# hydradarpa/kalman-hydra

Measured on AMD Instinct MI355X. Metric: frames/sec (Brox flow + EKF update) at 1024^2, higher is better.
Workload: dtype f32 (flow, renders) / f64 (EKF sums and state)

## Files before the change

include/hydra_mi.h:

```cpp
#ifndef HYDRA_MI_H
#define HYDRA_MI_H

#include <stdint.h>

#ifdef __cplusplus
extern "C" {
#endif

#define HM_OK 0
#define HM_ERR_ARG (-1)
#define HM_ERR_HIP (-2)
#define HM_ERR_STATE (-3)
#define HM_ERR_NUMERIC (-4)

const char *hm_last_error(void);
const char *hm_version(void);
int hm_device_count(void);

int hm_dev_alloc(int device, uint64_t bytes, void **out);
int hm_dev_free(int device, void *ptr);
int hm_dev_upload(int device, void *dst, const void *src, uint64_t bytes);
int hm_dev_download(int device, void *dst, const void *src, uint64_t bytes);
int hm_copy_stream_create(int device, void **stream_out);
int hm_copy_stream_destroy(int device, void *stream);
// ... 88 lines not shown
int hm_ms_newton_finish(void *worker, double *X, int *newton_iterations);
int hm_ms_worker_attach(void *worker, hm_ctx_t ctx);
int hm_newton_dev_start(hm_ctx_t h, int N, int n_bars, const int32_t *bars, const double *l0, double kappa, double M,
                        double dt, int maxiter, double tol, const double *X);
int hm_newton_dev_finish(hm_ctx_t h, double *X, int *newton_iterations);
int hm_update_arm_newton(hm_ctx_t h, void *worker, int n_bars, const int32_t *bars, const double *l0, double kappa,
                         double M, double dt, int maxiter, double tol);
int hm_update_arm_cov(hm_ctx_t h, double eps_F);
int hm_predict_take(hm_ctx_t h, const double *X, int n_bars, const int32_t *bars, const double *l0, double kappa,
                    double a, double s, double eps_F);
int hm_cov_predict(hm_ctx_t h, const double *W_in, int n_bars, const int32_t *bars, const double *blocks,
                   double a, double s, double eps_F, double *W_out);
int hm_ms_predict(hm_ctx_t h, int n_bars, const int32_t *bars, const double *l0, double kappa, double M, double dt,
                  int maxiter, double tol, double eps_F, double *X, int *newton_iterations, int prefactor);
int hm_update_last_error(hm_ctx_t h, const double *X, double err[4]);
int hm_chain_project(hm_ctx_t h);
int hm_prepare_mask(hm_ctx_t h, const uint8_t *d_y_m);
int hm_update_arm_mask(hm_ctx_t h, const uint8_t *d_y_m);
int hm_update_tail(hm_ctx_t h, double *Hzc, double *gains);
int hm_chain_states(hm_ctx_t h, double *predicted, double *projected, int *newton_iterations, int *moved);
int hm_ctx_tune(hm_ctx_t h, const char *key, int value);
int hm_ctx_tune64(hm_ctx_t h, const char *key, int64_t value);
int hm_ctx_sync(hm_ctx_t h);
void *hm_ctx_stream(hm_ctx_t h);

typedef struct hm_smooth *hm_smooth_t;
int hm_smooth_create(hm_ctx_t ctx, int capacity, int n_bars, const int32_t *bars, const double *l0, double kappa,
                     double a, double s, double eps_F, hm_smooth_t *out);
int hm_smooth_destroy(hm_smooth_t sm);
int hm_smooth_record(hm_smooth_t sm, const double *X);
// ... 142 lines not shown
```

kalman-hydra_amd/_lib.py:

```python
import ctypes
import os

import numpy as np

_HERE = os.path.dirname(os.path.abspath(__file__))
SO_PATH = os.environ.get("HYDRA_MI_SO") or os.path.join(_HERE, "libhydra_mi.so")

c_f32p = ctypes.POINTER(ctypes.c_float)
c_f64p = ctypes.POINTER(ctypes.c_double)
c_u8p = ctypes.POINTER(ctypes.c_uint8)
c_i32p = ctypes.POINTER(ctypes.c_int32)
c_vp = ctypes.c_void_p

SIGNATURES = {
    "hm_last_error": (ctypes.c_char_p, []),
    "hm_version": (ctypes.c_char_p, []),
    "hm_device_count": (ctypes.c_int, []),
    "hm_dev_alloc": (ctypes.c_int, [ctypes.c_int, ctypes.c_uint64, ctypes.POINTER(c_vp)]),
    "hm_dev_free": (ctypes.c_int, [ctypes.c_int, c_vp]),
    "hm_dev_upload": (ctypes.c_int, [ctypes.c_int, c_vp, c_vp, ctypes.c_uint64]),
    "hm_dev_download": (ctypes.c_int, [ctypes.c_int, c_vp, c_vp, ctypes.c_uint64]),
    "hm_copy_stream_create": (ctypes.c_int, [ctypes.c_int, ctypes.POINTER(c_vp)]),
    "hm_copy_stream_destroy": (ctypes.c_int, [ctypes.c_int, c_vp]),
    "hm_copy_stream_sync": (ctypes.c_int, [ctypes.c_int, c_vp]),
# ... 39 lines not shown
    "hm_render": (ctypes.c_int, [c_vp, c_vp, c_vp, c_vp, c_vp, c_vp]),
    "hm_initjacobian": (ctypes.c_int, [c_vp, c_vp, ctypes.c_int]),
    "hm_jz": (ctypes.c_int, [c_vp, c_vp, ctypes.c_int, c_f64p, c_f64p]),
    "hm_j": (ctypes.c_int, [c_vp, c_vp, ctypes.c_double, ctypes.c_int, ctypes.c_int, c_f64p]),
    "hm_jz_multi": (ctypes.c_int, [c_vp, c_vp, ctypes.c_int, c_vp, ctypes.c_int, c_vp, c_vp]),
    "hm_j_multi": (ctypes.c_int, [c_vp, c_vp, ctypes.c_double, ctypes.c_int, c_vp, c_vp, ctypes.c_int, c_vp, c_vp, c_vp]),
    "hm_error": (ctypes.c_int, [c_vp, c_vp, ctypes.c_int, c_f64p, c_vp, c_vp]),
    "hm_measure": (ctypes.c_int, [c_vp, c_vp, ctypes.c_double, ctypes.c_int, c_vp, c_vp, c_vp]),
    "hm_update_begin": (ctypes.c_int, [c_vp, c_vp, c_vp]),
    "hm_update_step": (ctypes.c_int, [c_vp, c_vp, ctypes.c_double, ctypes.c_int, c_vp, c_vp, c_f64p]),
    "hm_update_cov": (ctypes.c_int, [c_vp, ctypes.c_int, c_vp]),
    "hm_update_prefactor": (ctypes.c_int, [c_vp]),
    "hm_update_run": (ctypes.c_int, [c_vp, c_vp, c_vp, ctypes.c_double, ctypes.c_int, ctypes.c_int, ctypes.c_double,
                                     ctypes.POINTER(ctypes.c_int), c_vp, c_vp, c_vp, c_vp]),
    "hm_update_last_error": (ctypes.c_int, [c_vp, c_vp, c_f64p]),
    "hm_cov_fetch": (ctypes.c_int, [c_vp, c_vp]),
    "hm_project_mask": (ctypes.c_int, [c_vp, c_vp, c_vp, c_vp]),
    "hm_cov_predict": (ctypes.c_int, [c_vp, c_vp, ctypes.c_int, c_vp, c_vp, ctypes.c_double, ctypes.c_double,
                                      ctypes.c_double, c_vp]),
    "hm_ms_newton": (ctypes.c_int, [ctypes.c_int, ctypes.c_int, c_vp, c_vp, ctypes.c_double, ctypes.c_double,
                                    ctypes.c_double, ctypes.c_int, ctypes.c_double, c_vp, ctypes.POINTER(ctypes.c_int)]),
    "hm_ms_worker_create": (ctypes.c_int, [ctypes.POINTER(c_vp)]),
    "hm_ms_worker_destroy": (ctypes.c_int, [c_vp]),
    "hm_ms_newton_start": (ctypes.c_int, [c_vp, ctypes.c_int, ctypes.c_int, c_vp, c_vp, ctypes.c_double, ctypes.c_double,
                                          ctypes.c_double, ctypes.c_int, ctypes.c_double, c_vp]),
    "hm_ms_newton_finish": (ctypes.c_int, [c_vp, c_vp, ctypes.POINTER(ctypes.c_int)]),
    "hm_ms_worker_attach": (ctypes.c_int, [c_vp, c_vp]),
    "hm_newton_dev_start": (ctypes.c_int, [c_vp, ctypes.c_int, ctypes.c_int, c_vp, c_vp, ctypes.c_double, ctypes.c_double,
                                           ctypes.c_double, ctypes.c_int, ctypes.c_double, c_vp]),
    "hm_newton_dev_finish": (ctypes.c_int, [c_vp, c_vp, ctypes.POINTER(ctypes.c_int)]),
# ... 223 lines not shown
```

kalman-hydra_amd/csrc/ctx.h:

```cpp
#pragma once
#include "hm_common.h"
#include "hm_types.h"
#include "host_block.h"
#include <chrono>
#include <cmath>
#include <condition_variable>
#include <functional>
#include <mutex>
#include <thread>
#include <vector>

struct Helper {
    std::thread th;
    std::mutex m;
    std::condition_variable cv;
    std::function<int()> job;
    bool posted = false, busy = false, quit = false;
    int rc = HM_OK;
    char err[512] = "";
    void run()
    {
        std::unique_lock<std::mutex> lk(m);
        for (;;) {
            cv.wait(lk, [&] { return quit || posted; });
// ... 273 lines not shown
    Armed armed;
    hipEvent_t ev_m0 = nullptr;
    bool upd_open = false;
    bool prefactored = false;
    bool last_err_valid = false;
    double last_err[4] = {0, 0, 0, 0};
    std::vector<double> last_err_X;
    long long run_ticket = 0;
    std::thread worker;
    bool worker_active = false;
    int worker_rc = HM_OK;
    char worker_err[512] = "";
    int chol_flow = 1, flow_wgs = 192;
    int flow_stall = 0;
    int speculate = 1;
    double *d_flowP = nullptr;
    unsigned *d_flowctl = nullptr;
    MaskState mask;
    Newton4State newton4;
    NewtonState newton;
    ChainState chain;
    SpringState sp;
    ArmedPrediction pn;
    QueuedPrediction pq;
    TailState tail;
    MultiState multi;
    ViewState view;
    BodyState body;
    StrainState strain;
    RecState rec;
// ... 134 lines not shown
        const int a = bars[2 * i], b = bars[2 * i + 1];
        const double dx = X[2 * a] - X[2 * b], dy = X[2 * a + 1] - X[2 * b + 1];
        const double l = std::sqrt(dx * dx + dy * dy);
        const double k = kappa * (1.0 - l0[i] / l), c = kappa * l0[i] / (l * l * l);
        blk[3 * i] = k + c * dx * dx; blk[3 * i + 1] = c * dx * dy; blk[3 * i + 2] = k + c * dy * dy;
    }
}

__attribute__((visibility("hidden"))) void ekf_queue_setup_all(hipStream_t st, const Mesh &m, const double *d_X, TriSetup *d_setup);
__attribute__((visibility("hidden"))) void ekf_queue_render(hipStream_t st, const Mesh &m, const double *d_X, const TriSetup *d_setup,
                                                            const Targets &out, const int *d_labels, int *d_ids);
__attribute__((visibility("hidden"))) int render_iter(hm_ctx *h, const double *dX, Targets t, bool with_err, int masked, bool regions, double deltaX);
__attribute__((visibility("hidden"))) int render_strips(const hm_ctx *h);
__attribute__((visibility("hidden"))) int render_error_sums(hm_ctx *h, const char *who, double err[4]);
__attribute__((visibility("hidden"))) int measure_dev(hm_ctx *h, const double *dX, bool ref_ready, double deltaX, int masked,
                                                      bool regions_ready = false, bool scatter = true);
__attribute__((visibility("hidden"))) int measure_on_device(hm_ctx *h, const double *X, double deltaX, int masked, bool scatter = true);
__attribute__((visibility("hidden"))) int queue_star_regions(hm_ctx *h, const double *dX, double deltaX, int masked);
__attribute__((visibility("hidden"))) int pool_grow(hm_ctx *h, const char *who);
__attribute__((visibility("hidden"))) int prior_inverse(hm_ctx *h, const double *W_prior, hipStream_t st = nullptr);
#ifdef HM_STAMP
__attribute__((visibility("hidden"))) int update_debug_stamps(long long *dev_ptr);
#endif
__attribute__((visibility("hidden"))) int ensure_stream2(hm_ctx *h);
__attribute__((visibility("hidden"))) int queue_outline(hm_ctx *h, const uint8_t *mask);
__attribute__((visibility("hidden"))) int prepare_mask(hm_ctx *h, const uint8_t *d_y_m);
__attribute__((visibility("hidden"))) int queue_predict_ahead(hm_ctx *h, const double *X, int n_bars, const int32_t *bars, const double *l0,
                                                              double kappa, double M, double dt, double eps_F, hipStream_t st);

static inline int pool_flag_queue(hm_ctx *h)
{
// ... 24 lines not shown
```

kalman-hydra_amd/csrc/dense_kernels.h:

```cpp
#pragma once
#include <hip/hip_runtime.h>
#include "hm_types.h"
#include "host_block.h"

#define TTT_PF 3

__device__ __forceinline__ double d_rsqrt(double d)
{
    const double r = __builtin_amdgcn_rsq(d);
    const double e = fma(-(d * r), r, 1.0);
#ifdef HM_RSQRT_ORDER2
    return fma(r * 0.5, e, r);
#else
    return fma(r, fma(e, 0.375, 0.5) * e, r);
#endif
}

__device__ __forceinline__ double d_readlane(double v, int lane)
{
    const int lo = __builtin_amdgcn_readlane(__double2loint(v), lane);
    const int hi = __builtin_amdgcn_readlane(__double2hiint(v), lane);
    return __hiloint2double(hi, lo);
}

// ... 449 lines not shown
            for (int j = threadIdx.x; j < n; j += 256) A[(size_t)row * n + j] = 0.0;
        return;
    }
    double acc = 0.0;
    for (int j = threadIdx.x; j < n; j += 256) {
        const double h = H[(size_t)row * n + j];
        A[(size_t)row * n + j] = invW0[(size_t)row * n + j] + h;
        acc += h * (X0[j] + -1.0 * X[j]);
    }
    for (int o = 32; o > 0; o >>= 1) acc += __shfl_down(acc, o, 64);
    if ((threadIdx.x & 63) == 0) s[threadIdx.x >> 6] = acc;
    __syncthreads();
    if (threadIdx.x == 0) A[(size_t)rhs_row * n + row] = Hz[row] - (((s[0] + s[1]) + s[2]) + s[3]);
}


__global__ __launch_bounds__(256) void k_iter_result(const double *__restrict__ step, int n, const double *__restrict__ partial,
                                                     int ntiles, const int *__restrict__ overflow,
                                                     const unsigned *__restrict__ flow_ctl, double *__restrict__ res, double ticket,
                                                     int delay_us)
{
    __shared__ double sp[RI_GROUPS * RI_NV];
    __shared__ double sums[RI_NV];
    const int t = threadIdx.x;
    const unsigned long long stamp = hb_stamp((long long)ticket);
    d_tile_partial_sums(partial, ntiles, sp, sums);
    __syncthreads();
    double v = 0.0;
    int slot = -1;
    if (t < 4) { slot = t; v = sums[t]; }
    else if (t == 4) { slot = 4; v = (double)*overflow; }
    else if (t == 5) { slot = 5; v = ticket; }
    else if (t == 6) { slot = 6; v = 0.0; }
    else if (t == 7) { slot = 7; v = (double)flow_ctl[1]; }
    else if (t == 8) { slot = 8; v = sums[4]; }
    else if (t == 9) { slot = 9; v = sums[5]; }
    if (delay_us > 0) {
        if (t == 9) { hb_put(res, n + 9, v, stamp); hb_flush(); }
        hb_delay(delay_us);
    }
    for (int i = t; i < n; i += 256) hb_put(res, i, step[i], stamp);
    if (slot >= 0) hb_put(res, n + slot, v, stamp);
    hb_flush();
}

__global__ __launch_bounds__(256) void k_gains(const double *__restrict__ W, const double *__restrict__ Hzc, int n,
                                               double *__restrict__ out)
{
    __shared__ double sm[3][4];
    const int row = blockIdx.x;
    double a0 = 0.0, a1 = 0.0, a2 = 0.0;
    for (int j = threadIdx.x; j < n; j += 256) {
        const double w = W[(size_t)row * n + j];
        const double *c = Hzc + (size_t)4 * j;
        a0 += w * c[0];
        a1 += w * (c[1] + c[2]);
// ... 81 lines not shown
```

kalman-hydra_amd/csrc/ekf.hip:

```cpp
#include "ctx.h"
#include "ekf_kernels.h"
#include <algorithm>
#include <cmath>
#include <cstring>
#include <set>
#include <utility>
#include <vector>

static hipError_t pool_alloc(hm_ctx *h, long long cap)
{
    const size_t pc = (size_t)cap;
    h->pool.cap = 0;
    hipError_t e = h->own.grow(&h->pool.live, (pc / 64 + 1) * sizeof(int));
    for (short2 **q : {&h->pool.xi, &h->pool.yi})
        if (e == hipSuccess) e = h->own.grow(q, pc * sizeof(short2));
    for (float **q : {&h->pool.xfx, &h->pool.xfy, &h->pool.yfx, &h->pool.yfy, &h->pool.vxfx, &h->pool.vyfy})
        if (e == hipSuccess) e = h->own.grow(q, pc * sizeof(float));
    if (e == hipSuccess) h->pool.cap = cap;
    return e;
}
int pool_grow(hm_ctx *h, const char *who)
{
    std::vector<int> area(h->N);
    HM_HIP(hipMemcpyAsync(area.data(), h->d_area, (size_t)h->N * sizeof(int), hipMemcpyDeviceToHost, h->stream));
// ... 144 lines not shown
        dev(&h->d_Wprior, nn);
        dev(&h->d_gain, n4 * 3 * sizeof(double));
        h->pin_n = 2 * (n4 + RES_HEAD + n4 * 4 + n4 * 3) + 2;
        if (e == hipSuccess) e = h->own.host_alloc(&h->pin, h->pin_n * sizeof(double), hipHostMallocCoherent);
        if (e == hipSuccess) memset(h->pin, 0, h->pin_n * sizeof(double));
        h->pin_scratch = (int *)(h->pin + h->pin_n - 2);
        h->resv.assign(n4 + RES_HEAD, 0.0);
        h->tail.v.assign(n4 * 7, 0.0);
        dev(&h->d_X0, n4 * sizeof(double));
        dev(&h->pool.hdr, (size_t)4 * N * sizeof(int));
        dev(&h->pool.overflow, sizeof(int));
        dev(&h->d_area, (size_t)N * sizeof(int));
        h->pool.area = h->d_area;
        if (e == hipSuccess) e = pool_alloc(h, (long long)8 * W * H);
        dev(&h->d_Xn, n4 * sizeof(double));
        for (Targets *t : {&h->ref, &h->P, &h->Q})
            if (e == hipSuccess) e = alloc_targets(h->own, *t, n);
    }
    if (e != hipSuccess) {
        hm_set_error("hm_ctx_create: device allocation failed: %s", hipGetErrorString(e));
        step(HM_ERR_HIP);
    }
    if (rc != HM_OK) {
        ctx_free(h);
        return rc;
    }
    h->h_partial.resize((size_t)h->red_blocks * 4);
    h->h_tpart.resize((size_t)h->ntiles * RI_NV);
    *out = h;
    return HM_OK;
// ... 29 lines not shown
    int step;
    void (*set)(hm_ctx *, long long);
    const char *must;
} tune_keys[] = {
    {"measure_split", 1, MEAS_VSPLIT_MAX, 1, TUNE_SET(vsplit), nullptr},
    {"edge_split", 1, MEAS_VSPLIT_MAX, 1, TUNE_SET(esplit), nullptr},
    {"chol_flow", 0, 1, 1, TUNE_SET(chol_flow), "must be 0 (one launch per block step) or 1 (one persistent launch)"},
    {"chol_flow_wgs", 2, 2048, 1, TUNE_SET(flow_wgs), "must be in 2..2048 (the chain workgroup and at least one task workgroup)"},
    {"render_rows", 8, 16, 8, TUNE_SET(render_rows), "must be 8 or 16"},
    {"chol_flow_stall", 0, 100000, 1, TUNE_SET(flow_stall), nullptr},
    {"result_delay", 0, 5000, 1, TUNE_SET(result_delay), "must be in 0..5000 (microseconds)"},
    {"tail_async", 0, 1, 1, TUNE_SET(tail.async), "must be 0 or 1"},
    {"tail_split", 0, 1, 1, TUNE_SET(tail.split), "must be 0 or 1"},
    {"newton_fail", 0, 1, 1, TUNE_SET(newton4.fail), "must be 0 or 1"},
    {"speculate", 0, 1, 1, TUNE_SET(speculate), "must be 0 or 1"},
    {"body_stats_cap", 1, BODY_STATS_CAP, 1, TUNE_SET(body.stats_cap), nullptr},
    {"deep_col_entries", DEEP_COL_ENTRIES_MIN, DEEP_COL_ENTRIES_MAX, 1, TUNE_SET(body.deep_col_entries), nullptr},
    {"body_rec_chunk", 0, INT32_MAX, 1, TUNE_SET(rec.chunk), "must be >= 0 (0: the default size)"},
    {"rec_tp_frames", 1, REC_TP_MAX, 1, TUNE_SET(rec.tp_frames), nullptr},
    {"rec_bl_frames", 1, REC_BL_MAX, 1, TUNE_SET(rec.bl_frames), nullptr},
    {"rec_res_frames", 1, REC_RES_MAX, 1, TUNE_SET(rec.res_frames), nullptr},
    {"rec_map_frames", 1, REC_MAP_MAX, 1, TUNE_SET(rec.map_frames), nullptr},
    {"rec_null_frames", 1, REC_NULL_MAX, 1, TUNE_SET(rec.null_frames), nullptr},
    {"rec_tm_frames", 1, REC_TM_MAX, 1, TUNE_SET(rec.tm_frames), nullptr},
    {"rec_gram_bytes", 64, REC_GRAM_BYTES_MAX, 64, TUNE_SET(rec.gram_bytes), "must be a multiple of 64 in 64..131008"},
    {"rec_scratch_bytes", 1, 1 << 30, 1, TUNE_SET(rec.scr_bytes), nullptr},
    {"rec_ev_bytes", 1, 1ll << 34, 1, TUNE_SET(rec.ev_bytes), nullptr},
};
#undef TUNE_SET
static const TuneKey *tune_find(const char *key)
// ... 122 lines not shown
    a.ref = h->ref;
    a.obs = obs_of(h, masked);
    a.X = dX;
    a.delta = deltaX;
    a.out = h->d_out;
    a.pool = h->pool;
    a.vsplit = h->vsplit;
    a.esplit = h->esplit;
    a.iZ = 1.0 / h->eps_Z; a.iJ = 1.0 / h->eps_J; a.iM = 1.0 / h->eps_M;
    a.cfgs = h->d_cfgs;
    a.ubox = h->d_ubox;
    a.tmask = h->d_tmask;
    a.tlist = h->d_tlist;
    a.tcount = h->d_tcount;
    a.tmask_stride = TMASK_STRIDE;
}

static int state_upload(hm_ctx *h, const double *X)
{
    HM_HIP(hipMemcpyAsync(h->d_X, X, (size_t)4 * h->N * sizeof(double), hipMemcpyHostToDevice, h->stream));
    return HM_OK;
}

static int render_dev(hm_ctx *h, const double *dX, Targets t)
{
    const Mesh m = mesh_of(h);
    hipLaunchKernelGGL(k_setup_all, dim3(hm_cdiv(h->T, 64)), dim3(64), 0, h->stream, m, dX, h->d_setup);
    hipLaunchKernelGGL((k_render<0>), dim3(hm_cdiv(h->W, EKF_TILE), hm_cdiv(h->H, EKF_TILE)), dim3(EKF_TILE, EKF_TILE), 0,
                       h->stream, m, dX, h->d_setup, t, (const int *)nullptr, (int *)nullptr);
    HM_HIP(hipGetLastError());
// ... 275 lines not shown
    const int n = h->W * h->H;
    if (fx) HM_HIP(hipMemcpyAsync(fx, h->P.fx, (size_t)n * sizeof(float), hipMemcpyDeviceToHost, h->stream));
    if (fy) HM_HIP(hipMemcpyAsync(fy, h->P.fy, (size_t)n * sizeof(float), hipMemcpyDeviceToHost, h->stream));
    return render_error_sums(h, "hm_error", err);
}

int queue_star_regions(hm_ctx *h, const double *dX, double deltaX, int masked)
{
    MeasureArgs a;
    measure_args(h, dX, deltaX, masked, a);
    hipLaunchKernelGGL(k_star_regions, dim3(h->N), dim3(REGION_NT), 0, h->stream, a, h->d_area);
    HM_HIP(hipGetLastError());
    return HM_OK;
}

int measure_dev(hm_ctx *h, const double *dX, bool ref_ready, double deltaX, int masked, bool regions_ready, bool scatter)
{
    if (!ref_ready) {
        HM_TRY(render_iter(h, dX, h->ref, false, masked, !regions_ready, deltaX));
        regions_ready = true;
    }
    MeasureArgs a;
    measure_args(h, dX, deltaX, masked, a);
    if (!regions_ready) hipLaunchKernelGGL(k_star_regions, dim3(h->N), dim3(REGION_NT), 0, h->stream, a, h->d_area);
    hipLaunchKernelGGL(k_measure_vertex, dim3(h->N, h->vsplit), dim3(MEAS_NT), 0, h->stream, a,
                       (const TriSetup *)h->d_cfgs, (const int4 *)h->d_ubox, (const unsigned *)h->d_tmask);
    if (h->E > 0) hipLaunchKernelGGL(k_measure_edge, dim3(h->E, h->esplit), dim3(MEAS_NT), 0, h->stream, a);
    if (scatter) {
        ScatterArgs s = {h->d_out, h->d_edges, h->N, h->E, h->vsplit, h->esplit, h->eps_Z, h->eps_J, h->eps_M, deltaX, h->d_HTH, h->d_Hz, h->d_Hzc};
        hipLaunchKernelGGL(k_hth_scatter, dim3(hm_cdiv(h->njobs, 4)), dim3(256), 0, h->stream, s);
    }
    HM_HIP(hipGetLastError());
    return HM_OK;
}

int measure_on_device(hm_ctx *h, const double *X, double deltaX, int masked, bool scatter)
{
    HM_TRY(state_upload(h, X));
    h->X0.assign(X, X + 4 * h->N);
// ... 26 lines not shown
```

kalman-hydra_amd/csrc/ekf_kernels.h:

```cpp
#pragma once
#include <hip/hip_runtime.h>
#include <stdint.h>
#include "hm_types.h"

__global__ void k_setup_all(Mesh m, const double *__restrict__ X, TriSetup *__restrict__ out)
{
    int t = blockIdx.x * blockDim.x + threadIdx.x;
    if (t >= m.T) return;
    int v0 = m.tri[3 * t], v1 = m.tri[3 * t + 1], v2 = m.tri[3 * t + 2];
    TriSetup s;
    d_tri_setup(s, v0, v1, v2, d_snap(X[2 * v0]), d_snap(X[2 * v0 + 1]), d_snap(X[2 * v1]), d_snap(X[2 * v1 + 1]),
                d_snap(X[2 * v2]), d_snap(X[2 * v2 + 1]), m.W, m.H);
    d_tri_attr(s, m.uv, X, m.N);
    out[t] = s;
}

template <int MODE>
__global__ __launch_bounds__(EKF_TILE *EKF_TILE) void k_render(Mesh m, const double *__restrict__ X,
                                                                const TriSetup *__restrict__ setup, Targets out,
                                                                const int *__restrict__ labels, int *__restrict__ ids)
{
    __shared__ unsigned s_mask[EKF_MAX_TRI / 32];
    const int tid = threadIdx.y * EKF_TILE + threadIdx.x;
    const int words = (m.T + 31) / 32;
// ... 310 lines not shown
    StarTopo topo;
    Targets ref;
    Obs obs;
    const double *X;
    double delta;
    double *out;
    DPool pool;
    int vsplit;
    int esplit;
    double iZ, iJ, iM;
    TriSetup *cfgs;
    int4 *ubox;
    unsigned *tmask;
    int *tlist, *tcount;
    int tmask_stride;
};

#define MEAS_NT 256

#define MEAS_NCFG 5
#define UBOX_STRIDE (EKF_MAX_STAR + 4)
#define TMASK_STRIDE 1024

__device__ inline void d_vertex_cfgs(TriSetup (*cfg)[EKF_MAX_STAR + 1], int nsv, const int *trv, const Mesh &m,
                                     const double *X, int v, double d, int nthreads)
{
    const int wv = threadIdx.x >> 6, lane = threadIdx.x & 63, nw = nthreads >> 6;
    const double dxs[MEAS_NCFG] = {0, d, -d, 0, 0}, dys[MEAS_NCFG] = {0, 0, 0, d, -d};
    for (int c = wv; c < MEAS_NCFG; c += nw) d_star_setups(cfg[c], nsv, trv, m, X, v, dxs[c], dys[c], lane, 64);
}
// ... 137 lines not shown
        a += __shfl_down(a, o, 64); b += __shfl_down(b, o, 64); c += __shfl_down(c, o, 64);
    }
    const int lane = threadIdx.x & 63, wv = threadIdx.x >> 6;
    if (lane == 0) { s[wv * 3] = a; s[wv * 3 + 1] = b; s[wv * 3 + 2] = c; }
    __syncthreads();
    bv = 0; bw = 0; tot = 0;
    for (int k = 0; k < NT / 64; k++) { bv += s[k * 3]; bw += s[k * 3 + 1]; tot += s[k * 3 + 2]; }
}

#ifndef MEAS_OCC
#define MEAS_OCC 4
#endif
__global__ __launch_bounds__(MEAS_NT, MEAS_OCC) void k_measure_vertex(MeasureArgs a, const TriSetup *__restrict__ cfgs,
                                                                const int4 *__restrict__ ubox, const unsigned *__restrict__ tmask)
{
    __shared__ double s_red[(MEAS_NT / 64) * MEAS_OUT];
    __shared__ double s_k255[511];
    const double *k255 = s_k255 + 255;
    d_fill_k255(s_k255, MEAS_NT);
    const Mesh &m = a.m;
    const int N = m.N, W = m.W;
    const int v = blockIdx.x, job = v;
    const double *X = a.X;
    const double d = a.delta;
    const int nsv = a.topo.star_off[v + 1] - a.topo.star_off[v];
    const TriSetup *__restrict__ s_cfg[MEAS_NCFG];
#pragma unroll
    for (int c = 0; c < MEAS_NCFG; c++) s_cfg[c] = cfgs + ((size_t)v * MEAS_NCFG + c) * (EKF_MAX_STAR + 1);
    __syncthreads();
    const int c0 = a.pool.hdr[4 * v], r0 = a.pool.hdr[4 * v + 1], rw = a.pool.hdr[4 * v + 2], rh = a.pool.hdr[4 * v + 3];
// ... 100 lines not shown
struct EdgeTile {
    short2 ax, ay, bx, by;
    float axfx, axfy, ayfx, ayfy, avx, avy, bxfx, bxfy, byfx, byfy, bvx, bvy;
};
__device__ __forceinline__ EdgeTile d_edge_load(const DPool &P, long long pv, long long pw)
{
    EdgeTile t;
    t.ax = P.xi[pv]; t.bx = P.xi[pw]; t.ay = P.yi[pv]; t.by = P.yi[pw];
    t.axfx = P.xfx[pv]; t.axfy = P.xfy[pv]; t.ayfx = P.yfx[pv]; t.ayfy = P.yfy[pv]; t.avx = P.vxfx[pv]; t.avy = P.vyfy[pv];
    t.bxfx = P.xfx[pw]; t.bxfy = P.xfy[pw]; t.byfx = P.yfx[pw]; t.byfy = P.yfy[pw]; t.bvx = P.vxfx[pw]; t.bvy = P.vyfy[pw];
    return t;
}

__global__ __launch_bounds__(MEAS_NT) void k_measure_edge(MeasureArgs a)
{
    __shared__ double s_red[(MEAS_NT / 64) * MEAS_OUT];
    __shared__ double s_k255[511];
    const double *k255 = s_k255 + 255;
    d_fill_k255(s_k255, MEAS_NT);
    __syncthreads();
    const int N = a.m.N;
    const int e = blockIdx.x;
    const int v = a.topo.edges[2 * e], w = a.topo.edges[2 * e + 1];
    const int *hv = a.pool.hdr + 4 * v, *hw = a.pool.hdr + 4 * w;
    const int tx0 = max(hv[0], hw[0]) >> 3, ty0 = max(hv[1], hw[1]) >> 3;
    const int tx1 = min(hv[0] + hv[2], hw[0] + hw[2]) >> 3, ty1 = min(hv[1] + hv[3], hw[1] + hw[3]) >> 3;
    const int ntx = tx1 - tx0, nty = ty1 - ty0;
    const int vx0 = hv[0] >> 3, vy0 = hv[1] >> 3, vnx = hv[2] >> 3;
    const int wx0 = hw[0] >> 3, wy0 = hw[1] >> 3, wnx = hw[2] >> 3;
    __shared__ long long s_sum[(MEAS_NT / 64) * 3];
// ... 328 lines not shown
```

kalman-hydra_amd/csrc/hm_types.h:

```cpp
#pragma once
#include <hip/hip_runtime.h>
#include <stdint.h>
#include <stddef.h>


#define EKF_SUB 256
#define EKF_MAX_STAR 24
#define EKF_TILE 16
#define EKF_MAX_TRI 4096

struct TriSetup {
    double ea[3], eb[3], ec[3];
    double ecb[3];
    int cmin, cmax, rmin, rmax;
    int tl[3];
    float inv;
    int i0, i1, i2;
    float ux[3], uy[3], ax[3], ay[3];
};

__device__ __forceinline__ void d_tri_attr(TriSetup &s, const float *__restrict__ uv, const double *__restrict__ X, int N)
{
    const int id[3] = {s.i0, s.i1, s.i2};
    for (int k = 0; k < 3; k++) {
// ... 157 lines not shown
    A_XVY = 15, A_YVY = 16,
    A_VXVX = 17, A_VYVY = 18,
    A_NV = 19
};
enum {
    B_XX = 0, B_XY = 1, B_YX = 2, B_YY = 3,
    B_XVX = 4, B_YVX = 5, B_VXX = 6, B_VXY = 7, B_VXVX = 8,
    B_XVY = 9, B_YVY = 10, B_VYX = 11, B_VYY = 12, B_VYVY = 13,
    B_NV = 14
};
#define PREP_MAX_ENTRIES (4 * (EKF_MAX_STAR + 2))
#define RES_HEAD 10
#define RI_GROUPS 256
#define RI_NV 6

__device__ __forceinline__ void d_tile_partial_sums(const double *__restrict__ partial, int ntiles, double *sp, double *out)
{
    const int t = threadIdx.x;
    if (t < RI_GROUPS) {
        double s[RI_NV];
#pragma unroll
        for (int k = 0; k < RI_NV; k++) s[k] = 0.0;
#pragma unroll 4
        for (int i = t; i < ntiles; i += RI_GROUPS) {
            const double2 *q = (const double2 *)(partial + RI_NV * (size_t)i);
#pragma unroll
            for (int k = 0; k < RI_NV / 2; k++) { const double2 v = q[k]; s[2 * k] += v.x; s[2 * k + 1] += v.y; }
        }
#pragma unroll
        for (int k = 0; k < RI_NV; k++) sp[RI_NV * t + k] = s[k];
    }
    __syncthreads();
    if (t < RI_NV) {
        double s = 0.0;
        for (int g = 0; g < RI_GROUPS; g++) s += sp[RI_NV * g + t];
        out[t] = s;
    }
}

#define DNB 32

typedef double d4_t __attribute__((ext_vector_type(4)));

__device__ __forceinline__ d4_t d_mfma_nn(double (*X)[DNB + 1], double (*Y)[DNB + 1], int wv, int lane, d4_t c)
{
    const int i = 16 * (wv >> 1) + (lane & 15), j = 16 * (wv & 1) + (lane & 15), kq = lane >> 4;
#pragma unroll
    for (int kk = 0; kk < DNB / 4; kk++)
        c = __builtin_amdgcn_mfma_f64_16x16x4f64(X[i][4 * kk + kq], Y[4 * kk + kq][j], c, 0, 0, 0);
    return c;
}
__device__ __forceinline__ d4_t d_mfma_tn(double (*X)[DNB + 1], double (*Y)[DNB + 1], int wv, int lane, d4_t c)
// ... 94 lines not shown
```

kalman-hydra_amd/csrc/update.hip:

```cpp
#include "ctx.h"
#include "dense_kernels.h"
#include "chol_flow_kernels.h"
#include <algorithm>
#include <chrono>
#include <cmath>
#include <cstring>
#include <thread>
#include <utility>
#include <vector>

void ekf_queue_fpft(hipStream_t st, const double *src, double *FP, double *dst, int N, const SpringTopo &tp, double a, double s,
                    double eps_F)
{
    const dim3 grid(hm_cdiv(4 * N, 256), N);
    hipLaunchKernelGGL(k_fw_rows, grid, dim3(256), 0, st, src, FP, N, tp, a, s);
    hipLaunchKernelGGL(k_pft_cols, grid, dim3(256), 0, st, (const double *)FP, dst, N, tp, a, s, eps_F);
}
void ekf_queue_chol_flow(hipStream_t st, const FlowArgs &a, int wgs, bool fill)
{
    if (fill) hipLaunchKernelGGL(k_flow_fill, dim3(a.nrows + FLOW_FILL_WGS), dim3(256), 0, st, a);
    hipLaunchKernelGGL(k_chol_flow, dim3(wgs), dim3(FLOW_NT), 0, st, a);
}

#ifdef HM_STAMP
// ... 279 lines not shown
    double reltol;
    double *errs, *Hzc, *gains, *W_out;
};
struct UpdateRun {
    hm_ctx *const h;
    const UpdateArgs a;
    const Armed armed;
    const uint8_t *next_mask;
    const int n4;
    bool chained = false, collected = false;
    std::vector<double> X0, Xcur, Xold;
    int niter = 0, accepted = 0;
    bool reverted = false, conv = false;
    bool ref_ready = false;
    bool regions_ahead = false;
    bool measured_ahead = false;
    bool grown = false;
    double eold = 0.0;
    int slot = 0;
    bool dbg = false;
    std::chrono::steady_clock::time_point t_enter, t_queued;
    double stage[5] = {0, 0, 0, 0, 0};

    UpdateRun(hm_ctx *h, const UpdateArgs &a)
        : h(h), a(a), armed(std::exchange(h->armed, {})), next_mask(armed.mask), n4(4 * h->N) {}
    double ms() const { return std::chrono::duration<double, std::milli>(std::chrono::steady_clock::now() - t_enter).count(); }
    const double *res() const { return h->resv.data(); }
    double *pin_tail() const { return h->pin + 2 * ((size_t)n4 + RES_HEAD); }
};

struct SpecSwap {
// ... 26 lines not shown
    h->upd_X0 = u.X0;
    h->X0 = u.X0;
    u.collected = true;
    return HM_OK;
}

static int update_enter(UpdateRun &u)
{
    hm_ctx *h = u.h;
    h->tail.valid = false;
    HM_JOIN_LAZY(h);
    HM_ARG(u.a.deltaX > 0 && u.a.max_iter >= 0, "hm_update_run: deltaX must be positive, max_iter >= 0");
    u.chained = h->chain.pending;
    h->chain.pending = false;
    h->last_err_valid = false;
    h->pq.valid = false;
    h->tail.pending = false;
    NEED_TEX(h, "hm_update_run");
    NEED_OBS(h, "hm_update_run");
    u.dbg = getenv("HYDRA_MI_TRACE") != nullptr;
    u.t_enter = std::chrono::steady_clock::now();
    HM_TRY(update_begin(h, u.a.W_prior, u.chained ? nullptr : u.a.X));
    u.stage[0] = u.ms();
    u.collected = !u.chained;
    if (!u.chained) {
        u.X0.assign(u.a.X, u.a.X + u.n4); u.Xcur = u.X0; u.Xold = u.X0;
        HM_HIP(hipMemcpyAsync(h->d_X, h->d_X0, (size_t)u.n4 * sizeof(double), hipMemcpyDeviceToDevice, h->stream));
    }
    return HM_OK;
}
// ... 4 lines not shown
    if (!u.measured_ahead) HM_TRY(measure_dev(h, h->d_X, u.ref_ready, u.a.deltaX, u.a.masked, u.regions_ahead, false));
    u.measured_ahead = false;
    if (u.next_mask && it == 0) {
        HM_HIP(h->own.event(&h->ev_m0));
        HM_HIP(hipEventRecord(h->ev_m0, h->stream));
    }
    if (u.collected) h->X0 = u.Xcur;
    h->have_ref = true;
    u.slot = h->upd_last == 0 ? 1 : 0;
    HM_TRY(ctx_join(h));
    double *rhs_row = solve_step(h, u.slot, u.a.deltaX);
    u.regions_ahead = it + 1 < u.a.max_iter;
    HM_TRY(render_iter(h, h->d_Xn, h->P, true, u.a.masked, u.regions_ahead, u.a.deltaX));
    hipLaunchKernelGGL(k_iter_result, dim3(1), dim3(256), 0, h->stream, rhs_row, u.n4, h->d_tpart,
                       render_strips(h), h->pool.overflow, (const unsigned *)h->d_flowctl, h->pin, (double)(++h->run_ticket),
                       h->result_delay);
    HM_HIP(hipGetLastError());
    if (h->speculate && u.regions_ahead) {
        swap.set();
        u.measured_ahead = true;
        HM_TRY(measure_dev(h, h->d_X, true, u.a.deltaX, u.a.masked, true, false));
    }
    u.t_queued = std::chrono::steady_clock::now();
    return HM_OK;
}

static int update_meanwhile(UpdateRun &u, int it)
{
    hm_ctx *h = u.h;
    if (u.next_mask && it == 0) {
        HM_TRY(ensure_stream2(h));
        HM_HIP(hipStreamWaitEvent(h->stream2, h->ev_m0, 0));
        HM_TRY(prepare_mask(h, u.next_mask));
        u.next_mask = nullptr;
    }
    if (!u.collected) {
        const int rc = chain_collect(u);
        if (rc) { (void)hipStreamSynchronize(h->stream); return rc; }
    }
    return HM_OK;
}

enum class Taken { go_on, retry };
static int update_take_result(UpdateRun &u, int it, SpecSwap &swap, Taken *out)
{
    hm_ctx *h = u.h;
    const int n4 = u.n4;
    HM_TRY(hb_wait(h->stream, h->pin, 0, (size_t)n4 + RES_HEAD, hb_stamp(h->run_ticket), h->resv.data(), "hm_update_run"));
    if (u.dbg) {
        const double ms = std::chrono::duration<double, std::milli>(std::chrono::steady_clock::now() - u.t_queued).count();
        if (ms > 1.5) fprintf(stderr, "[hydra_mi] hm_update_run: iteration %d waited %.2f ms for its result\n", it, ms);
    }
    if (u.res()[n4 + 4] == 0.0) {
        u.grown = false;
        h->upd_prev = h->upd_last;
        h->upd_last = u.slot;
        u.niter++;
        *out = Taken::go_on;
        return HM_OK;
    }
    swap.undo();
    u.measured_ahead = false;
    if (u.grown) { hm_set_error("hm_update_run: the star regions do not fit the difference-image pool"); return HM_ERR_STATE; }
    if (u.regions_ahead) {
        HM_TRY(queue_star_regions(h, h->d_X, u.a.deltaX, u.a.masked));
    }
    HM_HIP(hipStreamSynchronize(h->stream));
    HM_TRY(pool_grow(h, "hm_update_run"));
    u.grown = true;
    u.regions_ahead = false;
    HM_HIP(hipMemsetAsync(h->d_flowctl, 0, 4 * sizeof(unsigned), h->stream));
    *out = Taken::retry;
    return HM_OK;
}

enum class Verdict { go_on, reverted, converged };
static int update_judge(UpdateRun &u, int it, Verdict *out)
// ... 2 lines not shown
    const int n4 = u.n4;
    const double *res = u.res();
    if (res[n4 + 7] != 0.0) {
        hm_set_error("hm_update_run: the factorisation launch gave up waiting for a block (chol_flow time-out)");
        return HM_ERR_HIP;
    }
    bool finite = true;
    for (int i = 0; i < n4; i++) finite = finite && std::isfinite(res[i]);
    if (!finite) {
        hm_set_error("hm_update_run: the update system inv(W) + HTH is not positive definite "
                     "(non-finite state, covariance or observation?)");
        return HM_ERR_NUMERIC;
    }
    for (int i = 0; i < n4; i++) u.Xcur[i] = u.X0[i] + res[i];
    if (u.a.errs) for (int k = 0; k < 4; k++) u.a.errs[4 * it + k] = res[n4 + k];
    bool flipped = false;
    for (int t = 0; t < h->T && !flipped; t++) {
        const int a = h->tri[3 * t], b = h->tri[3 * t + 1], c = h->tri[3 * t + 2];
        const double ax = u.Xcur[2 * b] - u.Xcur[2 * a], ay = u.Xcur[2 * b + 1] - u.Xcur[2 * a + 1];
        const double bx = u.Xcur[2 * c] - u.Xcur[2 * a], by = u.Xcur[2 * c + 1] - u.Xcur[2 * a + 1];
        flipped = ax * by - ay * bx < 0.0;
    }
    if (flipped) {
        u.Xcur = u.Xold;
        u.reverted = true;
        *out = Verdict::reverted;
        return HM_OK;
    }
    const double e_im = std::trunc(res[n4]), e_m = std::trunc(res[n4 + 3]);
    const double enew = std::sqrt(e_im * e_im + res[n4 + 1] * res[n4 + 1] + res[n4 + 2] * res[n4 + 2] + e_m * e_m);
    u.accepted++;
    if (std::fabs(enew - u.eold) / enew < u.a.reltol) {
        u.conv = true;
        *out = Verdict::converged;
        return HM_OK;
    }
    u.eold = enew;
    u.Xold = u.Xcur;
    u.ref_ready = true;
    h->X0 = u.Xcur;
    *out = Verdict::go_on;
    return HM_OK;
}

static int update_state_final(UpdateRun &u)
{
    hm_ctx *h = u.h;
// ... 114 lines not shown
extern "C" int hm_update_run(hm_ctx_t h, const double *W_prior, double *X, double deltaX, int masked, int max_iter,
                             double reltol, int info[4], double *errs, double *Hzc, double *gains, double *W_out)
{
    HM_ARG(h && X && info, "hm_update_run: NULL argument");
    UpdateRun u(h, {W_prior, X, deltaX, masked, max_iter, reltol, errs, Hzc, gains, W_out});
    HM_TRY(update_enter(u));
    for (int it = 0; it < max_iter;) {
        SpecSwap swap(h);
        HM_TRY(update_queue_iteration(u, it, swap));
        HM_TRY(update_meanwhile(u, it));
        Taken taken = Taken::go_on;
        HM_TRY(update_take_result(u, it, swap, &taken));
        if (taken == Taken::retry) continue;
        Verdict verdict = Verdict::go_on;
        HM_TRY(update_judge(u, it, &verdict));
        if (verdict != Verdict::go_on) break;
        swap.keep();
        it++;
    }
    HM_TRY(update_state_final(u));
    HM_TRY(update_tail(u));
    update_finish(u, info);
    return HM_OK;
}

extern "C" int hm_update_last_error(hm_ctx_t h, const double *X, double err[4])
{
    HM_ARG(h && X && err, "hm_update_last_error: NULL argument");
    if (!h->last_err_valid || h->last_err_X.size() != (size_t)4 * h->N) return 1;
    if (memcmp(X, h->last_err_X.data(), (size_t)4 * h->N * sizeof(double)) != 0) return 1;
    for (int k = 0; k < 4; k++) err[k] = h->last_err[k];
    return HM_OK;
}
```

kalman-hydra_amd/renderer.py:

```python
import ctypes
import os

import numpy as np

from . import _lib
from . import matio
from .readout import Readout
from .record import Record


class ChainedPredictionFailed(RuntimeError):
    """hm_update_run, chained to a state prediction on the device (hm_chain_project), found that the prediction's inner
    solve had given up: nothing was updated; predict on the host and update again."""


class Renderer(Readout, Record):
    def __init__(self, distmesh, vel, flow, nx, im1, cuda, eps_Z, eps_J, eps_M, labels=None, labels_hess=None,
                 Q=None, showtracking=False, force=None, multi=True, device=0):
        if not cuda:
            raise NotImplementedError(
                "cuda=False: this build has no CPU measurement path (the reference's NumPy twin, "
                "cuda.py:929-1010, is restated under oracle/ as test infrastructure only)")
        self._h = None
        self.Q = Q
# ... 287 lines not shown
        self._worker = None

    def chain_project(self):
        rc = _lib.lib().hm_chain_project(self._h)
        if rc == 1:
            return False
        _lib.check(rc, "hm_chain_project")
        return True

    def update_tail(self):
        n4 = 4 * self.n
        Hzc, gains = np.empty((n4, 4)), np.empty((3, n4))
        _lib.check(_lib.lib().hm_update_tail(self._h, _lib.ptr(Hzc), _lib.ptr(gains)), "hm_update_tail")
        return Hzc, gains

    def arm_mask(self, d_mask):
        _lib.check(_lib.lib().hm_update_arm_mask(self._h, ctypes.c_void_p(int(d_mask))), "hm_update_arm_mask")

    def prepare_mask(self, d_mask):
        p = None if d_mask is None else ctypes.c_void_p(int(d_mask))
        _lib.check(_lib.lib().hm_prepare_mask(self._h, p), "hm_prepare_mask")

    def chain_states(self):
        n4 = 4 * self.n
        pred, proj = np.empty(n4), np.empty(n4)
        its, moved = ctypes.c_int(0), ctypes.c_int(0)
        _lib.check(_lib.lib().hm_chain_states(self._h, _lib.ptr(pred), _lib.ptr(proj), ctypes.byref(its), ctypes.byref(moved)),
                   "hm_chain_states")
        return pred, proj, its.value, moved.value

# ... 125 lines not shown
```

Baseline: 331.9.

## Gate speculative measurement on a device-computed continue verdict

```diff
diff --git a/include/hydra_mi.h b/include/hydra_mi.h
--- a/include/hydra_mi.h
+++ b/include/hydra_mi.h
@@ -126,6 +126,9 @@
 int hm_ms_predict(hm_ctx_t h, int n_bars, const int32_t *bars, const double *l0, double kappa, double M, double dt,
                   int maxiter, double tol, double eps_F, double *X, int *newton_iterations, int prefactor);
 int hm_update_last_error(hm_ctx_t h, const double *X, double err[4]);
+int hm_update_spec_stats(hm_ctx_t h, int out[4]);
+int hm_update_verdict(int N, int T, const int32_t *tri, const double *X0, const double *step, const double sums[4],
+                      double eold, double reltol, double *enew);
 int hm_chain_project(hm_ctx_t h);
 int hm_prepare_mask(hm_ctx_t h, const uint8_t *d_y_m);
 int hm_update_arm_mask(hm_ctx_t h, const uint8_t *d_y_m);
diff --git a/kalman-hydra_amd/_lib.py b/kalman-hydra_amd/_lib.py
--- a/kalman-hydra_amd/_lib.py
+++ b/kalman-hydra_amd/_lib.py
@@ -77,6 +77,9 @@
     "hm_update_run": (ctypes.c_int, [c_vp, c_vp, c_vp, ctypes.c_double, ctypes.c_int, ctypes.c_int, ctypes.c_double,
                                      ctypes.POINTER(ctypes.c_int), c_vp, c_vp, c_vp, c_vp]),
     "hm_update_last_error": (ctypes.c_int, [c_vp, c_vp, c_f64p]),
+    "hm_update_spec_stats": (ctypes.c_int, [c_vp, ctypes.POINTER(ctypes.c_int)]),
+    "hm_update_verdict": (ctypes.c_int, [ctypes.c_int, ctypes.c_int, c_vp, c_vp, c_vp, c_vp, ctypes.c_double, ctypes.c_double,
+                                         c_f64p]),
     "hm_cov_fetch": (ctypes.c_int, [c_vp, c_vp]),
     "hm_project_mask": (ctypes.c_int, [c_vp, c_vp, c_vp, c_vp]),
     "hm_cov_predict": (ctypes.c_int, [c_vp, c_vp, ctypes.c_int, c_vp, c_vp, ctypes.c_double, ctypes.c_double,
diff --git a/kalman-hydra_amd/csrc/ctx.h b/kalman-hydra_amd/csrc/ctx.h
--- a/kalman-hydra_amd/csrc/ctx.h
+++ b/kalman-hydra_amd/csrc/ctx.h
@@ -311,6 +311,9 @@
     int chol_flow = 1, flow_wgs = 192;
     int flow_stall = 0;
     int speculate = 1;
+    int spec_gate = 1;
+    int *d_gate = nullptr;
+    int spec_stats[4] = {0, 0, 0, 0};
     double *d_flowP = nullptr;
     unsigned *d_flowctl = nullptr;
     MaskState mask;
@@ -475,7 +478,7 @@
 __attribute__((visibility("hidden"))) int render_strips(const hm_ctx *h);
 __attribute__((visibility("hidden"))) int render_error_sums(hm_ctx *h, const char *who, double err[4]);
 __attribute__((visibility("hidden"))) int measure_dev(hm_ctx *h, const double *dX, bool ref_ready, double deltaX, int masked,
-                                                      bool regions_ready = false, bool scatter = true);
+                                                      bool regions_ready = false, bool scatter = true, const int *gate = nullptr);
 __attribute__((visibility("hidden"))) int measure_on_device(hm_ctx *h, const double *X, double deltaX, int masked, bool scatter = true);
 __attribute__((visibility("hidden"))) int queue_star_regions(hm_ctx *h, const double *dX, double deltaX, int masked);
 __attribute__((visibility("hidden"))) int pool_grow(hm_ctx *h, const char *who);
diff --git a/kalman-hydra_amd/csrc/dense_kernels.h b/kalman-hydra_amd/csrc/dense_kernels.h
--- a/kalman-hydra_amd/csrc/dense_kernels.h
+++ b/kalman-hydra_amd/csrc/dense_kernels.h
@@ -487,25 +487,47 @@
     if (threadIdx.x == 0) A[(size_t)rhs_row * n + row] = Hz[row] - (((s[0] + s[1]) + s[2]) + s[3]);
 }
 
+#define IR_PRE 2
+#define IR_TRI_LANES 192
 
 __global__ __launch_bounds__(256) void k_iter_result(const double *__restrict__ step, int n, const double *__restrict__ partial,
                                                      int ntiles, const int *__restrict__ overflow,
                                                      const unsigned *__restrict__ flow_ctl, double *__restrict__ res, double ticket,
-                                                     int delay_us)
+                                                     int delay_us, const double *__restrict__ X0, const int *__restrict__ tri, int T,
+                                                     double eold, double reltol, int gate_mode, int *__restrict__ gate)
 {
     __shared__ double sp[RI_GROUPS * RI_NV];
     __shared__ double sums[RI_NV];
-    const int t = threadIdx.x;
+    __shared__ int s_stop[4];
+    const int t = threadIdx.x, tl = t - 64;
     const unsigned long long stamp = hb_stamp((long long)ticket);
-    d_tile_partial_sums(partial, ntiles, sp, sums);
+    int pre[3 * IR_PRE];
+#pragma unroll
+    for (int k = 0; k < IR_PRE; k++) {
+        const int tt = tl + IR_TRI_LANES * k;
+        const bool in = tl >= 0 && tt < T;
+#pragma unroll
+        for (int q = 0; q < 3; q++) pre[3 * k + q] = in ? tri[3 * tt + q] : 0;
+    }
+    const int ovf = *overflow;
+    const unsigned timed_out = flow_ctl[1];
+    d_tile_partial_groups(partial, ntiles, sp);
+    __syncthreads();
+    if (tl < 0) {
+        d_tile_partial_total(sp, sums);
+    } else {
+        int stop = hm_iter_verdict(X0, step, tri, tl, IR_TRI_LANES, T, pre, IR_PRE, nullptr, 0.0, 0.0, nullptr);
+        for (int i = tl; i < n; i += IR_TRI_LANES) stop |= isfinite(step[i]) ? 0 : 1;
+        const unsigned long long any = __ballot(stop != 0);
+        if ((t & 63) == 0) s_stop[t >> 6] = any != 0 ? 1 : 0;
+    }
     __syncthreads();
     double v = 0.0;
     int slot = -1;
     if (t < 4) { slot = t; v = sums[t]; }
-    else if (t == 4) { slot = 4; v = (double)*overflow; }
+    else if (t == 4) { slot = 4; v = (double)ovf; }
     else if (t == 5) { slot = 5; v = ticket; }
-    else if (t == 6) { slot = 6; v = 0.0; }
-    else if (t == 7) { slot = 7; v = (double)flow_ctl[1]; }
+    else if (t == 7) { slot = 7; v = (double)timed_out; }
     else if (t == 8) { slot = 8; v = sums[4]; }
     else if (t == 9) { slot = 9; v = sums[5]; }
     if (delay_us > 0) {
@@ -513,6 +535,15 @@
         hb_delay(delay_us);
     }
     for (int i = t; i < n; i += 256) hb_put(res, i, step[i], stamp);
+    if (t == IR_TRI_LANES) {
+        double enew;
+        const int conv = hm_iter_verdict(X0, step, tri, T, 1, T, nullptr, 0, sums, eold, reltol, &enew) & HM_V_CONVERGED;
+        int go = !(conv || s_stop[1] || s_stop[2] || s_stop[3] || ovf != 0 || timed_out != 0);
+        if (gate_mode == 2) go = 0;
+        else if (gate_mode != 1) go = 1;
+        *gate = go;
+        slot = 6; v = (double)go;
+    }
     if (slot >= 0) hb_put(res, n + slot, v, stamp);
     hb_flush();
 }
diff --git a/kalman-hydra_amd/csrc/ekf.hip b/kalman-hydra_amd/csrc/ekf.hip
--- a/kalman-hydra_amd/csrc/ekf.hip
+++ b/kalman-hydra_amd/csrc/ekf.hip
@@ -182,6 +182,8 @@
         h->pool.area = h->d_area;
         if (e == hipSuccess) e = pool_alloc(h, (long long)8 * W * H);
         dev(&h->d_Xn, n4 * sizeof(double));
+        dev(&h->d_gate, sizeof(int));
+        if (e == hipSuccess) e = hipMemsetAsync(h->d_gate, 0, sizeof(int), h->stream);
         for (Targets *t : {&h->ref, &h->P, &h->Q})
             if (e == hipSuccess) e = alloc_targets(h->own, *t, n);
     }
@@ -241,6 +243,7 @@
     {"tail_split", 0, 1, 1, TUNE_SET(tail.split), "must be 0 or 1"},
     {"newton_fail", 0, 1, 1, TUNE_SET(newton4.fail), "must be 0 or 1"},
     {"speculate", 0, 1, 1, TUNE_SET(speculate), "must be 0 or 1"},
+    {"spec_gate", 0, 3, 1, TUNE_SET(spec_gate), "must be 0 (never gated), 1 (the device's hint), 2 (hint forced to stop) or 3 (forced to go)"},
     {"body_stats_cap", 1, BODY_STATS_CAP, 1, TUNE_SET(body.stats_cap), nullptr},
     {"deep_col_entries", DEEP_COL_ENTRIES_MIN, DEEP_COL_ENTRIES_MAX, 1, TUNE_SET(body.deep_col_entries), nullptr},
     {"body_rec_chunk", 0, INT32_MAX, 1, TUNE_SET(rec.chunk), "must be >= 0 (0: the default size)"},
@@ -393,6 +396,7 @@
     a.tlist = h->d_tlist;
     a.tcount = h->d_tcount;
     a.tmask_stride = TMASK_STRIDE;
+    a.gate = nullptr;
 }
 
 static int state_upload(hm_ctx *h, const double *X)
@@ -698,7 +702,8 @@
     return HM_OK;
 }
 
-int measure_dev(hm_ctx *h, const double *dX, bool ref_ready, double deltaX, int masked, bool regions_ready, bool scatter)
+int measure_dev(hm_ctx *h, const double *dX, bool ref_ready, double deltaX, int masked, bool regions_ready, bool scatter,
+                const int *gate)
 {
     if (!ref_ready) {
         HM_TRY(render_iter(h, dX, h->ref, false, masked, !regions_ready, deltaX));
@@ -707,6 +712,7 @@
     MeasureArgs a;
     measure_args(h, dX, deltaX, masked, a);
     if (!regions_ready) hipLaunchKernelGGL(k_star_regions, dim3(h->N), dim3(REGION_NT), 0, h->stream, a, h->d_area);
+    a.gate = gate;
     hipLaunchKernelGGL(k_measure_vertex, dim3(h->N, h->vsplit), dim3(MEAS_NT), 0, h->stream, a,
                        (const TriSetup *)h->d_cfgs, (const int4 *)h->d_ubox, (const unsigned *)h->d_tmask);
     if (h->E > 0) hipLaunchKernelGGL(k_measure_edge, dim3(h->E, h->esplit), dim3(MEAS_NT), 0, h->stream, a);
diff --git a/kalman-hydra_amd/csrc/ekf_kernels.h b/kalman-hydra_amd/csrc/ekf_kernels.h
--- a/kalman-hydra_amd/csrc/ekf_kernels.h
+++ b/kalman-hydra_amd/csrc/ekf_kernels.h
@@ -348,6 +348,7 @@
     unsigned *tmask;
     int *tlist, *tcount;
     int tmask_stride;
+    const int *gate;
 };
 
 #define MEAS_NT 256
@@ -515,6 +516,7 @@
 __global__ __launch_bounds__(MEAS_NT, MEAS_OCC) void k_measure_vertex(MeasureArgs a, const TriSetup *__restrict__ cfgs,
                                                                 const int4 *__restrict__ ubox, const unsigned *__restrict__ tmask)
 {
+    if (a.gate && *a.gate == 0) return;
     __shared__ double s_red[(MEAS_NT / 64) * MEAS_OUT];
     __shared__ double s_k255[511];
     const double *k255 = s_k255 + 255;
@@ -645,6 +647,7 @@
 
 __global__ __launch_bounds__(MEAS_NT) void k_measure_edge(MeasureArgs a)
 {
+    if (a.gate && *a.gate == 0) return;
     __shared__ double s_red[(MEAS_NT / 64) * MEAS_OUT];
     __shared__ double s_k255[511];
     const double *k255 = s_k255 + 255;
diff --git a/kalman-hydra_amd/csrc/hm_types.h b/kalman-hydra_amd/csrc/hm_types.h
--- a/kalman-hydra_amd/csrc/hm_types.h
+++ b/kalman-hydra_amd/csrc/hm_types.h
@@ -2,6 +2,7 @@
 #include <hip/hip_runtime.h>
 #include <stdint.h>
 #include <stddef.h>
+#include <math.h>
 
 
 #define EKF_SUB 256
@@ -195,7 +196,7 @@
 #define RI_GROUPS 256
 #define RI_NV 6
 
-__device__ __forceinline__ void d_tile_partial_sums(const double *__restrict__ partial, int ntiles, double *sp, double *out)
+__device__ __forceinline__ void d_tile_partial_groups(const double *__restrict__ partial, int ntiles, double *sp)
 {
     const int t = threadIdx.x;
     if (t < RI_GROUPS) {
@@ -211,12 +212,49 @@
 #pragma unroll
         for (int k = 0; k < RI_NV; k++) sp[RI_NV * t + k] = s[k];
     }
-    __syncthreads();
+}
+__device__ __forceinline__ void d_tile_partial_total(const double *sp, double *out)
+{
+    const int t = threadIdx.x;
     if (t < RI_NV) {
         double s = 0.0;
         for (int g = 0; g < RI_GROUPS; g++) s += sp[RI_NV * g + t];
         out[t] = s;
     }
+}
+__device__ __forceinline__ void d_tile_partial_sums(const double *__restrict__ partial, int ntiles, double *sp, double *out)
+{
+    d_tile_partial_groups(partial, ntiles, sp);
+    __syncthreads();
+    d_tile_partial_total(sp, out);
+}
+
+#define HM_V_FLIPPED 1
+#define HM_V_CONVERGED 2
+static inline __host__ __device__ int hm_iter_verdict(const double *X0, const double *step, const int *tri, int t0, int ts, int T,
+                                                      const int *pre, int npre, const double *sums, double eold, double reltol,
+                                                      double *enew)
+{
+#pragma clang fp contract(off)
+    int v = 0;
+    auto corner = [&](int a, int b, int c) {
+#pragma clang fp contract(off)
+        const double pax = X0[2 * a] + step[2 * a], pay = X0[2 * a + 1] + step[2 * a + 1];
+        const double ax = (X0[2 * b] + step[2 * b]) - pax, ay = (X0[2 * b + 1] + step[2 * b + 1]) - pay;
+        const double bx = (X0[2 * c] + step[2 * c]) - pax, by = (X0[2 * c + 1] + step[2 * c + 1]) - pay;
+        if (ax * by - ay * bx < 0.0) v |= HM_V_FLIPPED;
+    };
+#pragma unroll
+    for (int k = 0; k < npre; k++)
+        if (t0 + k * ts < T) corner(pre[3 * k], pre[3 * k + 1], pre[3 * k + 2]);
+    for (int t = t0 + npre * ts; t < T; t += ts) corner(tri[3 * t], tri[3 * t + 1], tri[3 * t + 2]);
+    if (sums) {
+        const double e_im = trunc(sums[0]), e_m = trunc(sums[3]);
+        const double e = sqrt(e_im * e_im + sums[1] * sums[1] + sums[2] * sums[2] + e_m * e_m);
+        if (fabs(e - eold) / e < reltol) v |= HM_V_CONVERGED;
+        *enew = e;
+    }
+    return v;
 }
 
 #define DNB 32
diff --git a/kalman-hydra_amd/csrc/update.hip b/kalman-hydra_amd/csrc/update.hip
--- a/kalman-hydra_amd/csrc/update.hip
+++ b/kalman-hydra_amd/csrc/update.hip
@@ -317,7 +317,7 @@
     bool reverted = false, conv = false;
     bool ref_ready = false;
     bool regions_ahead = false;
-    bool measured_ahead = false;
+    bool queued_ahead = false, measured_ahead = false;
     bool grown = false;
     double eold = 0.0;
     int slot = 0;
@@ -374,6 +374,7 @@
     u.chained = h->chain.pending;
     h->chain.pending = false;
     h->last_err_valid = false;
+    std::fill(h->spec_stats, h->spec_stats + 4, 0);
     h->pq.valid = false;
     h->tail.pending = false;
     NEED_TEX(h, "hm_update_run");
@@ -408,12 +409,15 @@
     HM_TRY(render_iter(h, h->d_Xn, h->P, true, u.a.masked, u.regions_ahead, u.a.deltaX));
     hipLaunchKernelGGL(k_iter_result, dim3(1), dim3(256), 0, h->stream, rhs_row, u.n4, h->d_tpart,
                        render_strips(h), h->pool.overflow, (const unsigned *)h->d_flowctl, h->pin, (double)(++h->run_ticket),
-                       h->result_delay);
+                       h->result_delay, (const double *)h->d_X0, (const int *)h->d_tri, h->T, u.eold, u.a.reltol, h->spec_gate,
+                       h->d_gate);
     HM_HIP(hipGetLastError());
+    u.queued_ahead = false;
     if (h->speculate && u.regions_ahead) {
         swap.set();
-        u.measured_ahead = true;
-        HM_TRY(measure_dev(h, h->d_X, true, u.a.deltaX, u.a.masked, true, false));
+        u.queued_ahead = true;
+        h->spec_stats[0]++;
+        HM_TRY(measure_dev(h, h->d_X, true, u.a.deltaX, u.a.masked, true, false, h->spec_gate ? h->d_gate : nullptr));
     }
     u.t_queued = std::chrono::steady_clock::now();
     return HM_OK;
@@ -433,6 +437,22 @@
         if (rc) { (void)hipStreamSynchronize(h->stream); return rc; }
     }
     return HM_OK;
+}
+
+static void spec_settle(UpdateRun &u, bool goes_on)
+{
+    hm_ctx *h = u.h;
+    u.measured_ahead = false;
+    if (!u.queued_ahead) return;
+    u.queued_ahead = false;
+    const bool ran = u.res()[u.n4 + 6] != 0.0;
+    if (!ran) {
+        h->spec_stats[1]++;
+        if (goes_on) h->spec_stats[3]++;
+    } else if (!goes_on) {
+        h->spec_stats[2]++;
+    }
+    u.measured_ahead = goes_on && ran;
 }
 
 enum class Taken { go_on, retry };
@@ -454,7 +474,7 @@
         return HM_OK;
     }
     swap.undo();
-    u.measured_ahead = false;
+    spec_settle(u, false);
     if (u.grown) { hm_set_error("hm_update_run: the star regions do not fit the difference-image pool"); return HM_ERR_STATE; }
     if (u.regions_ahead) {
         HM_TRY(queue_star_regions(h, h->d_X, u.a.deltaX, u.a.masked));
@@ -487,23 +507,16 @@
     }
     for (int i = 0; i < n4; i++) u.Xcur[i] = u.X0[i] + res[i];
     if (u.a.errs) for (int k = 0; k < 4; k++) u.a.errs[4 * it + k] = res[n4 + k];
-    bool flipped = false;
-    for (int t = 0; t < h->T && !flipped; t++) {
-        const int a = h->tri[3 * t], b = h->tri[3 * t + 1], c = h->tri[3 * t + 2];
-        const double ax = u.Xcur[2 * b] - u.Xcur[2 * a], ay = u.Xcur[2 * b + 1] - u.Xcur[2 * a + 1];
-        const double bx = u.Xcur[2 * c] - u.Xcur[2 * a], by = u.Xcur[2 * c + 1] - u.Xcur[2 * a + 1];
-        flipped = ax * by - ay * bx < 0.0;
-    }
-    if (flipped) {
+    double enew = 0.0;
+    const int v = hm_iter_verdict(u.X0.data(), res, h->tri.data(), 0, 1, h->T, nullptr, 0, res + n4, u.eold, u.a.reltol, &enew);
+    if (v & HM_V_FLIPPED) {
         u.Xcur = u.Xold;
         u.reverted = true;
         *out = Verdict::reverted;
         return HM_OK;
     }
-    const double e_im = std::trunc(res[n4]), e_m = std::trunc(res[n4 + 3]);
-    const double enew = std::sqrt(e_im * e_im + res[n4 + 1] * res[n4 + 1] + res[n4 + 2] * res[n4 + 2] + e_m * e_m);
     u.accepted++;
-    if (std::fabs(enew - u.eold) / enew < u.a.reltol) {
+    if (v & HM_V_CONVERGED) {
         u.conv = true;
         *out = Verdict::converged;
         return HM_OK;
@@ -648,6 +661,7 @@
         if (taken == Taken::retry) continue;
         Verdict verdict = Verdict::go_on;
         HM_TRY(update_judge(u, it, &verdict));
+        spec_settle(u, verdict == Verdict::go_on);
         if (verdict != Verdict::go_on) break;
         swap.keep();
         it++;
@@ -656,6 +670,21 @@
     HM_TRY(update_tail(u));
     update_finish(u, info);
     return HM_OK;
+}
+
+extern "C" int hm_update_spec_stats(hm_ctx_t h, int out[4])
+{
+    HM_ARG(h && out, "hm_update_spec_stats: NULL argument");
+    for (int k = 0; k < 4; k++) out[k] = h->spec_stats[k];
+    return HM_OK;
+}
+
+extern "C" int hm_update_verdict(int N, int T, const int32_t *tri, const double *X0, const double *step, const double sums[4],
+                                 double eold, double reltol, double *enew)
+{
+    HM_ARG(N >= 3 && T >= 0 && tri && X0 && step && sums && enew, "hm_update_verdict: bad argument");
+    for (int i = 0; i < 3 * T; i++) HM_ARG(tri[i] >= 0 && tri[i] < N, "hm_update_verdict: triangle %d refers to vertex %d (N=%d)", i / 3, tri[i], N);
+    return hm_iter_verdict(X0, step, tri, 0, 1, T, nullptr, 0, sums, eold, reltol, enew);
 }
 
 extern "C" int hm_update_last_error(hm_ctx_t h, const double *X, double err[4])
diff --git a/kalman-hydra_amd/renderer.py b/kalman-hydra_amd/renderer.py
--- a/kalman-hydra_amd/renderer.py
+++ b/kalman-hydra_amd/renderer.py
@@ -325,6 +325,11 @@
         _lib.check(_lib.lib().hm_update_tail(self._h, _lib.ptr(Hzc), _lib.ptr(gains)), "hm_update_tail")
         return Hzc, gains
 
+    def spec_stats(self):
+        out = (ctypes.c_int * 4)()
+        _lib.check(_lib.lib().hm_update_spec_stats(self._h, out), "hm_update_spec_stats")
+        return tuple(out[:])
+
     def arm_mask(self, d_mask):
         _lib.check(_lib.lib().hm_update_arm_mask(self._h, ctypes.c_void_p(int(d_mask))), "hm_update_arm_mask")
 
```

After: 334.1, median of 6. About the same (+0.7%).
